# wty-yy/go2_rl_gym

Hardware: AMD Instinct MI355X
Metric: env-steps/sec at 4096 envs (go2 flat); 1/2/4/8-GPU scaling (higher is better)
Workload: dtype f32; 1 GPU; task=go2 flat terrain (go2_flat), num_envs=4096 per GPU, full PPO iteration = 24 rollout steps + GAE + 5 epochs x 4 mini-batches; num_envs_per_gpu=4096, num_steps_per_env=24, parallelism=env-sharded dp1

## Files before the change

### go2_rl_gym_amd/csrc/go2nn_bx3.h

```cpp
#pragma once

#ifndef GO2_EMU
typedef __bf16 bf16x8 __attribute__((ext_vector_type(8)));
typedef __bf16 bf16x2 __attribute__((ext_vector_type(2)));
typedef unsigned u32x2 __attribute__((ext_vector_type(2)));
typedef unsigned u32x4 __attribute__((ext_vector_type(4)));
#endif

#define BX3_BK 16
#ifndef BX3_DA
#define BX3_DA(TM) ((TM) == 1 ? 4 : 2)
#endif
#define BX3_SGB_VALU 5
#define BX3_TILE_BYTES 12288

#ifdef GO2_EMU
#define BX3_HD
#else
#define BX3_HD __host__ __device__
#endif
BX3_HD static inline long long bx3_image_bytes(int rows, int con) { return (long long)((rows + 127) / 128) * ((con + BX3_BK - 1) / BX3_BK) * BX3_TILE_BYTES; }

struct Bx3Prob {
  const float* A; const unsigned char* B; float* C; const float* bias; const float* Y; float* part;
  int M, N, K, lda, ldc, nbm, nbn, c_vec, nkt;
  const float* Bf; int ldb;
  float* wpart; int kx;
};
struct Bx3Args { Bx3Prob p[2]; int ntiles0, ntiles; long long* stamps; int wg_M, wg_rows; };
struct Bx3SplitJob { const float* w; unsigned char* img; int N, K; };
struct Bx3SplitArgs { Bx3SplitJob j[GO2NN_MAX_SPLIT_JOBS]; int njobs; };

#ifndef GO2_EMU
__device__ __forceinline__ unsigned bx3_pk(float a, float b) { f32x2 v = {a, b}; return __builtin_bit_cast(unsigned, __builtin_convertvector(v, bf16x2)); }
__device__ __forceinline__ float bx3_lo(unsigned p) { return __builtin_bit_cast(float, p << 16); }
__device__ __forceinline__ float bx3_hi(unsigned p) { return __builtin_bit_cast(float, p & 0xffff0000u); }
__device__ __forceinline__ void bx3_split4(const f32x4& x, u32x2& h, u32x2& m, u32x2& l) {
  h[0] = bx3_pk(x[0], x[1]); h[1] = bx3_pk(x[2], x[3]);
  const float r0 = x[0] - bx3_lo(h[0]), r1 = x[1] - bx3_hi(h[0]), r2 = x[2] - bx3_lo(h[1]), r3 = x[3] - bx3_hi(h[1]);
  m[0] = bx3_pk(r0, r1); m[1] = bx3_pk(r2, r3);
  const float s0 = r0 - bx3_lo(m[0]), s1 = r1 - bx3_hi(m[0]), s2 = r2 - bx3_lo(m[1]), s3 = r3 - bx3_hi(m[1]);
  l[0] = bx3_pk(s0, s1); l[1] = bx3_pk(s2, s3);
}

__global__ void __launch_bounds__(256) go2nn_bx3_split_kernel(const Bx3SplitArgs sa) {
  const int job = blockIdx.y >> 1, tr = blockIdx.y & 1;
  const Bx3SplitJob& j = sa.j[job];
  const int rows = tr ? j.K : j.N, con = tr ? j.N : j.K;
  const int nrt = (rows + 127) / 128, nkt = (con + BX3_BK - 1) / BX3_BK;
  const long long id = (long long)blockIdx.x * 256 + threadIdx.x;
  if (id >= (long long)nrt * nkt * 256) return;
  const int chunk = (int)(id & 1), r = (int)(id >> 1) & 127, tile = (int)(id >> 8), kt = tile % nkt, rt = tile / nkt;
  const int row = rt * 128 + r, c0 = kt * BX3_BK + chunk * 8;
  f32x4 v[2];
#pragma unroll
  for (int e = 0; e < 8; ++e) {
    const int c = c0 + e;
    const bool in = row < rows && c < con;
    const int rr = min(row, rows - 1), cc = min(c, con - 1);
    const float x = tr ? j.w[(size_t)cc * j.K + rr] : j.w[(size_t)rr * j.K + cc];
    v[e >> 2][e & 3] = in ? x : 0.f;
  }
  u32x2 h0, m0, l0, h1, m1, l1;
  bx3_split4(v[0], h0, m0, l0); bx3_split4(v[1], h1, m1, l1);
  unsigned char* img = j.img + (tr ? bx3_image_bytes(j.N, j.K) : 0) + (size_t)tile * BX3_TILE_BYTES + r * 32 + ((chunk ^ ((r >> 3) & 1)) << 4);
  *reinterpret_cast<u32x4*>(img) = u32x4{h0[0], h0[1], h1[0], h1[1]};
  *reinterpret_cast<u32x4*>(img + 4096) = u32x4{m0[0], m0[1], m1[0], m1[1]};
  *reinterpret_cast<u32x4*>(img + 8192) = u32x4{l0[0], l0[1], l1[0], l1[1]};
}

__device__ __forceinline__ int lane_pos_x(int i, int gk) { return i * 2 + gk; }
template <int OFF> __device__ __forceinline__ void bx3_dsr128(u32x4& d, unsigned addr) { asm volatile("ds_read_b128 %0, %1 offset:%2" : "=v"(d) : "v"(addr), "i"(OFF) : "memory"); }
template <int TM> struct Bx3Frags {
  u32x4 a[TM][2], b[2][2];
  __device__ __forceinline__ void opaque() {
#pragma unroll
    for (int p = 0; p < 2; ++p) {
#pragma unroll
      for (int t = 0; t < TM; ++t) g3_opaque(a[t][p]);
#pragma unroll
      for (int t = 0; t < 2; ++t) g3_opaque(b[t][p]);
    }
  }
};
template <int TM, int EPI, bool WG = false>
__global__ void __launch_bounds__(256, 2) go2nn_bx3_kernel(const Bx3Args ga) {
  static_assert(!WG || (TM == 2 && EPI == EPI_STORE), "weight-gradient mode: 128 x 128 tiles, plain store");
  static_assert(EPI != EPI_DELU_WG || (TM == 2 && !WG), "input gradient + the weight gradient below: 128-row tiles");
  constexpr int BM = 64 * TM, BN = 128, BK = BX3_BK, TN = 2;
  constexpr int AP = BM * 32, BP = 4096, BOFF = 3 * AP, STAGE = 3 * AP + 3 * BP, LOOP_LDS = 2 * STAGE, EPI_LDS = 4 * 32 * 32 * TN * 4;
  using SA = G3Stage<BM, true, BK>;
  using FR = Bx3Frags<TM>;
  __shared__ __attribute__((aligned(16))) unsigned char lds[LOOP_LDS > EPI_LDS ? LOOP_LDS : EPI_LDS];
  const int tid = threadIdx.x, lane = tid & 63, wave = tid >> 6, i = lane & 31, gk = lane >> 5, wm = wave & 1, wn = wave >> 1;
  int t = blockIdx.x, pi, slice = 0;
  const int n0 = ga.ntiles0, n1 = ga.ntiles - ga.ntiles0;
  if constexpr (WG) {
    const int xcd = t & 7, idx = t >> 3;
    slice = (idx / ga.ntiles) * 8 + xcd; t = idx % ga.ntiles;
    pi = t >= n0 ? 1 : 0; t -= pi ? n0 : 0;
  } else if (((n0 | n1) & 7) == 0) { const int x = t & 7, j = t >> 3, c0 = n0 >> 3, c1 = n1 >> 3; pi = j >= c0 ? 1 : 0; t = pi ? x * c1 + (j - c0) : x * c0 + j; }
  else { pi = t >= n0 ? 1 : 0; t -= pi ? n0 : 0; }
  const Bx3Prob& g = ga.p[pi];
  const int bm = t / g.nbn, bn = t - bm * g.nbn;
  const int row0 = bm * BM, col0 = bn * BN;
  const int nk = WG ? (ga.wg_rows + BK - 1) / BK : g.nkt;
  const int m0 = slice * ga.wg_rows;
  float* const Cout = g.C + (WG ? (size_t)slice * g.M * g.N : 0);

#ifdef GM3_STAMPS
  long long st_[6] = {0, 0, 0, 0, 0, 0};
  const long long wall0_ = wall_clock64();
#endif
  G3_T(0);
  f32x16 acc[TM][TN];
#pragma unroll
  for (int a = 0; a < TM; ++a)
#pragma unroll
    for (int b = 0; b < TN; ++b)
#pragma unroll
      for (int r = 0; r < 16; ++r) acc[a][b][r] = 0.f;

  constexpr int CT = 32 * TN, LPR = CT / 4, RPI = 64 / LPR, NI = 32 / RPI;
  const int lc = (lane % LPR) * 4, lr = lane / LPR;
  const int col = col0 + wn * CT + lc;
  const bool cv = g.c_vec != 0 && col + 3 < g.N;
  float4 bias4 = make_float4(0.f, 0.f, 0.f, 0.f);
  if (EPI == EPI_BIAS_ELU || EPI == EPI_BIAS) {
    const int c1 = min(col, g.N - 1), c2 = min(col + 1, g.N - 1), c3 = min(col + 2, g.N - 1), c4 = min(col + 3, g.N - 1);
    bias4 = make_float4(g.bias[c1], g.bias[c2], g.bias[c3], g.bias[c4]);
  }
  float4 y4[EPI == EPI_DELU_COLSUM ? TM : 1][EPI == EPI_DELU_COLSUM ? NI : 1];
  auto load_y = [&](auto a_c) __attribute__((always_inline)) {
    constexpr int A_ = decltype(a_c)::value;
    if constexpr (EPI == EPI_DELU_COLSUM) {
#pragma unroll
      for (int n = 0; n < NI; ++n) {
        const float* q = g.Y + (size_t)min(row0 + wm * 32 * TM + A_ * 32 + lr + n * RPI, g.M - 1) * g.ldc;
        if (cv) y4[A_][n] = *reinterpret_cast<const float4*>(q + col);
        else y4[A_][n] = make_float4(q[min(col, g.N - 1)], q[min(col + 1, g.N - 1)], q[min(col + 2, g.N - 1)], q[min(col + 3, g.N - 1)]);
      }
    }
  };

  const int kx = EPI == EPI_DELU_WG ? g.kx : 0;
  const bool two = kx > 32;
  const int xj = tid & 31, xjt = (tid >> 5) & 1, xhk = (tid >> 6) & 1, xkb = tid >> 7;
  float xv[EPI == EPI_DELU_WG ? 4 : 1][8];
  auto issue_xv = [&]() __attribute__((always_inline)) {
    if constexpr (EPI == EPI_DELU_WG) {
      if (xjt == 0 || two) {
        const float* const xq = g.Bf + min(xjt * 32 + xj, kx - 1);
#pragma unroll
        for (int rt = 0; rt < 4; ++rt)
#pragma unroll
          for (int e = 0; e < 8; ++e) xv[rt][e] = xq[(size_t)gm_opaque(min(row0 + rt * 32 + 16 * xkb + (e & 3) + 8 * (e >> 2) + 4 * xhk, g.M - 1)) * g.ldb];
      }
    }
  };
  SA sa; sa.init(g.A, g.lda, row0, g.M, WG ? 4 : g.K, tid);
  constexpr int DA = BX3_DA(TM);
  f32x4 ba[DA][WG ? 4 : SA::P]; u32x4 bb[3];
  const int scol = tid & 127, skg = tid >> 7;
  unsigned voa[WG ? 8 : 1], vob[WG ? 8 : 1];
  if constexpr (WG) {
#pragma unroll
    for (int j = 0; j < 8; ++j) {
      voa[j] = (unsigned)(((skg * 8 + j) * g.lda + row0 + scol) * 4);
      vob[j] = col0 + scol < g.N ? (unsigned)(((skg * 8 + j) * g.ldb + col0 + scol) * 4) : 0x7ffffff0u;
    }
  }
  auto wg_rsrc = [&](const float* base, int ld, int mrow) __attribute__((always_inline)) {
    const long long left = (long long)(ga.wg_M - mrow) * ld * 4;
    const float* p0 = base + (size_t)mrow * ld;
    const unsigned lo = __builtin_amdgcn_readfirstlane((unsigned)(uintptr_t)p0), hi = __builtin_amdgcn_readfirstlane((unsigned)((uintptr_t)p0 >> 32));
    const unsigned nb = __builtin_amdgcn_readfirstlane(left > 0 ? (unsigned)(left < 0x7fffffe0ll ? left : 0x7fffffe0ll) : 0u);
    return __builtin_amdgcn_make_buffer_rsrc(reinterpret_cast<void*>(((uintptr_t)hi << 32) | lo), 0, nb, 0x00020000);
  };
  auto issue_wg = [&](int kt, f32x4 (&w)[WG ? 4 : SA::P]) __attribute__((always_inline)) {
    if constexpr (WG) {
      const int mrow = m0 + kt * BK;
      const auto ra = wg_rsrc(g.A, g.lda, mrow), rb = wg_rsrc(g.Bf, g.ldb, mrow);
#pragma unroll
      for (int j = 0; j < 8; ++j) {
        w[j >> 2][j & 3] = __builtin_bit_cast(float, __builtin_amdgcn_raw_buffer_load_b32(ra, voa[j], 0, 0));
        w[2 + (j >> 2)][j & 3] = __builtin_bit_cast(float, __builtin_amdgcn_raw_buffer_load_b32(rb, vob[j], 0, 0));
      }
    }
  };
  auto commit_wg = [&](int stage, int kt, const f32x4 (&w)[WG ? 4 : SA::P]) __attribute__((always_inline)) {
    if constexpr (WG) {
      unsigned char* st = lds + stage * STAGE + scol * 32 + ((skg ^ ((scol >> 3) & 1)) << 4);
      const f32x4 a0 = w[0], a1 = w[1];
      u32x2 h0, m0_, l0, h1, m1, l1;
      bx3_split4(a0, h0, m0_, l0); bx3_split4(a1, h1, m1, l1);
      *reinterpret_cast<u32x4*>(st) = u32x4{h0[0], h0[1], h1[0], h1[1]};
      *reinterpret_cast<u32x4*>(st + AP) = u32x4{m0_[0], m0_[1], m1[0], m1[1]};
      *reinterpret_cast<u32x4*>(st + 2 * AP) = u32x4{l0[0], l0[1], l1[0], l1[1]};
      bx3_split4(w[2], h0, m0_, l0); bx3_split4(w[3], h1, m1, l1);
      *reinterpret_cast<u32x4*>(st + BOFF) = u32x4{h0[0], h0[1], h1[0], h1[1]};
      *reinterpret_cast<u32x4*>(st + BOFF + BP) = u32x4{m0_[0], m0_[1], m1[0], m1[1]};
      *reinterpret_cast<u32x4*>(st + BOFF + 2 * BP) = u32x4{l0[0], l0[1], l1[0], l1[1]};
    }
  };
  const unsigned char* bimg = WG ? nullptr : g.B + (size_t)bn * nk * BX3_TILE_BYTES + tid * 16;
  auto issue_b = [&](int kt) __attribute__((always_inline)) {
    if constexpr (WG) return;
    const unsigned char* s = bimg + (size_t)kt * BX3_TILE_BYTES;
#pragma unroll
    for (int p = 0; p < 3; ++p) bb[p] = *reinterpret_cast<const u32x4*>(s + p * 4096);
  };
  const int kq = tid & 3, srow = tid >> 2;
  const unsigned st_off = (unsigned)(srow * 32 + (((kq >> 1) ^ ((srow >> 3) & 1)) << 4) + ((kq & 1) << 3));
  auto commit = [&](auto fix_c, int stage, int kt, const f32x4 (&ba)[SA::P]) __attribute__((always_inline)) {
    constexpr bool FIX = decltype(fix_c)::value;
    unsigned char* st = lds + stage * STAGE;
#pragma unroll
    for (int p = 0; p < SA::P; ++p) {
      f32x4 v = ba[p];
      if (FIX) {
        const int k = kt * BK + sa.lead, sh = k - min(k, g.K - 4);
#pragma unroll
        for (int e = 0; e < 4; ++e) { float tv = 0.f;
#pragma unroll
          for (int q = 0; q < 4; ++q) tv = (q == e + sh) ? ba[p][q] : tv;
          v[e] = k + e < g.K ? tv : 0.f; }
      }
      u32x2 h, m, l; bx3_split4(v, h, m, l);
      unsigned char* d = st + st_off + p * (64 * 32);
      *reinterpret_cast<u32x2*>(d) = h; *reinterpret_cast<u32x2*>(d + AP) = m; *reinterpret_cast<u32x2*>(d + 2 * AP) = l;
    }
#pragma unroll
    for (int p = 0; p < 3; ++p) *reinterpret_cast<u32x4*>(st + BOFF + p * 4096 + tid * 16) = bb[p];
  };
  const unsigned lbase = (unsigned)(uintptr_t)lds;
  const unsigned fch = (unsigned)((gk ^ ((i >> 3) & 1)) << 4);
  const unsigned fa = lbase + (unsigned)((wm * 32 * TM + i) * 32) + fch, fb = lbase + (unsigned)(BOFF + (wn * 64 + i) * 32) + fch;
  FR f0, f1; u32x4 la[TM], lb[2];
  auto read_frags = [&](auto stage_c, FR& f) __attribute__((always_inline)) {
    constexpr int SOFF = decltype(stage_c)::value * STAGE;
    g3_for<0, TM>([&](auto a_c) __attribute__((always_inline)) { constexpr int A = decltype(a_c)::value; bx3_dsr128<SOFF + 2 * AP + A * 32 * 32>(la[A], fa); });
    g3_for<0, 2>([&](auto b_c) __attribute__((always_inline)) { constexpr int B = decltype(b_c)::value; bx3_dsr128<SOFF + 2 * BP + B * 32 * 32>(lb[B], fb); });
    g3_for<0, 2>([&](auto p_c) __attribute__((always_inline)) {
      constexpr int P = decltype(p_c)::value;
      g3_for<0, TM>([&](auto a_c) __attribute__((always_inline)) { constexpr int A = decltype(a_c)::value; bx3_dsr128<SOFF + P * AP + A * 32 * 32>(f.a[A][P], fa); });
      g3_for<0, 2>([&](auto b_c) __attribute__((always_inline)) { constexpr int B = decltype(b_c)::value; bx3_dsr128<SOFF + P * BP + B * 32 * 32>(f.b[B][P], fb); });
    });
  };
  auto mfmas = [&](auto q0_c, auto q1_c, const FR& f) __attribute__((always_inline)) {
    constexpr int PA[6] = {2, 0, 1, 1, 0, 0}, PB[6] = {0, 2, 1, 0, 1, 0};
    g3_for<decltype(q0_c)::value, decltype(q1_c)::value>([&](auto q_c) __attribute__((always_inline)) {
      constexpr int Q = decltype(q_c)::value;
#pragma unroll
      for (int a = 0; a < TM; ++a)
#pragma unroll
        for (int b = 0; b < TN; ++b) {
          const u32x4 av = PA[Q] == 2 ? la[a] : f.a[a][PA[Q] & 1], bv = PB[Q] == 2 ? lb[b] : f.b[b][PB[Q] & 1];
          acc[a][b] = __builtin_amdgcn_mfma_f32_32x32x16_bf16(__builtin_bit_cast(bf16x8, av), __builtin_bit_cast(bf16x8, bv), acc[a][b], 0, 0, 0);
        }
    });
  };
  auto lo_opaque = [&]() __attribute__((always_inline)) {
#pragma unroll
    for (int t = 0; t < TM; ++t) g3_opaque(la[t]);
#pragma unroll
    for (int t = 0; t < 2; ++t) g3_opaque(lb[t]);
  };

  const bool ragged = !WG && (g.K & (BK - 1)) != 0;
  const int nkp = ragged ? nk - 1 : nk;
  auto tile = [&](auto cur_c, auto set_c, const bool MORE, int kt) __attribute__((always_inline)) {
    constexpr int CUR = decltype(cur_c)::value, SET = decltype(set_c)::value;
    auto& a_ld = ba[SET]; auto& a_st = ba[(SET + 1) % DA];
    FR& fc = CUR ? f1 : f0; FR& fn = CUR ? f0 : f1;
    { const int k2 = min(kt + DA, nkp - 1); if constexpr (WG) issue_wg(k2, a_ld); else sa.issue(k2 * BK, a_ld); }
    g3_wait_lgkm<0>();
    fc.opaque(); lo_opaque();
    mfmas(G3Int<0>{}, G3Int<3>{}, fc);
    if (MORE) {
      if constexpr (WG) commit_wg(CUR ^ 1, kt + 1, a_st); else commit(G3Int<0>{}, CUR ^ 1, kt + 1, a_st);
      issue_b(min(kt + 2, nkp - 1));
#pragma unroll
      for (int q = 0; q < 6 * TM; ++q) {
        __builtin_amdgcn_sched_group_barrier(0x008, 1, 0);
        __builtin_amdgcn_sched_group_barrier(0x002, BX3_SGB_VALU, 0);
        __builtin_amdgcn_sched_group_barrier(0x200, 1, 0);
        if (q < 3) __builtin_amdgcn_sched_group_barrier(0x020, 1, 0);
      }
      __builtin_amdgcn_sched_barrier(0);
      __syncthreads();
      read_frags(G3Int<CUR ^ 1>{}, fn);
      __builtin_amdgcn_sched_barrier(0);
    }
    mfmas(G3Int<3>{}, G3Int<6>{}, fc);
    __builtin_amdgcn_sched_barrier(0);
  };
  constexpr G3Int<0> I0{}; constexpr G3Int<1> I1{};
  if (nkp > 0) {
    issue_b(0);
    g3_for<0, DA>([&](auto d_c) __attribute__((always_inline)) { constexpr int D_ = decltype(d_c)::value;
      if constexpr (WG) issue_wg(min(D_, nkp - 1), ba[D_]); else sa.issue(min(D_, nkp - 1) * BK, ba[D_]); });
    if constexpr (TM == 2) load_y(G3Int<0>{});
    issue_xv();
    if constexpr (WG) commit_wg(0, 0, ba[0]); else commit(I0, 0, 0, ba[0]);
    if (nkp > 1) issue_b(1);
    __syncthreads();
    read_frags(I0, f0);
    G3_T(1);
    constexpr int G = (DA % 2) ? 2 * DA : DA;
    for (int kt = 0; kt < nkp; kt += G)
      g3_for<0, G>([&](auto j_c) __attribute__((always_inline)) { constexpr int J = decltype(j_c)::value; if (kt + J < nkp) tile(G3Int<J & 1>{}, G3Int<J % DA>{}, kt + J + 1 < nkp, kt + J); });
  } else if constexpr (TM == 2) {
    issue_xv();
    load_y(G3Int<0>{});
  }
  if constexpr (!WG) if (ragged) {
    __syncthreads();
    sa.issue((nk - 1) * BK, ba[0]); issue_b(nk - 1);
    commit(I1, 0, nk - 1, ba[0]);
    __syncthreads();
    read_frags(I0, f0);
    g3_wait_lgkm<0>();
    f0.opaque(); lo_opaque();
    mfmas(G3Int<0>{}, G3Int<6>{}, f0);
  }
  G3_T(2);
  __syncthreads();
  G3_T(3);

  if constexpr (EPI == EPI_DELU_WG) {
#if defined(GM3_STAMPS) && defined(WG_T3)
#define WG_STAMP(n) do { if (WG_T3 == (n)) G3_T(3); if (WG_T5 == (n)) G3_T(5); } while (0)
#else
#define WG_STAMP(n) do { } while (0)
#endif
    const int rw = row0 + wm * 64, cw = col0 + wn * 64;
    const bool xon = xjt == 0 || two;
    float y[2][2][16];
#pragma unroll
    for (int a = 0; a < 2; ++a)
#pragma unroll
      for (int r = 0; r < 16; ++r) {
        const float* q = g.Y + (size_t)gm_opaque(min(rw + a * 32 + (r & 3) + 8 * (r >> 2) + 4 * gk, g.M - 1)) * g.ldc;
#pragma unroll
        for (int b = 0; b < 2; ++b) y[a][b][r] = q[min(cw + b * 32 + i, g.N - 1)];
      }
    WG_STAMP(1);
    float cs[2] = {0.f, 0.f};
#pragma unroll
    for (int a = 0; a < 2; ++a)
#pragma unroll
      for (int r = 0; r < 16; ++r) {
        const bool in = rw + a * 32 + (r & 3) + 8 * (r >> 2) + 4 * gk < g.M;
#pragma unroll
        for (int b = 0; b < 2; ++b) {
          const float v = gm_keep(acc[a][b][r] * (y[a][b][r] > 0.f ? 1.f : y[a][b][r] + 1.f), in);
          acc[a][b][r] = v; cs[b] += v;
        }
      }
#pragma unroll
    for (int b = 0; b < 2; ++b) {
      const float t2 = cs[b] + __shfl_xor(cs[b], 32);
      const int c = cw + b * 32 + i;
      if (gk == 0 && c < g.N && (bm * 2 + wm) * 64 < g.M) g.part[(size_t)(bm * 2 + wm) * g.N + c] = t2;
    }
    if (g.C) {
      float* wl = reinterpret_cast<float*>(lds) + wave * (32 * CT);
#pragma unroll
      for (int a = 0; a < 2; ++a) {
#pragma unroll
        for (int b = 0; b < 2; ++b)
#pragma unroll
          for (int r = 0; r < 16; ++r) {
            const int row = (r & 3) + 8 * (r >> 2) + 4 * gk, cc = b * 32 + i;
            wl[row * CT + (cc ^ (gk << 5 & (CT - 1)))] = acc[a][b][r];
          }
#pragma unroll
        for (int n = 0; n < NI; ++n) {
          const int lrow = lr + n * RPI, row = rw + a * 32 + lrow;
          const float4 v = *reinterpret_cast<const float4*>(wl + lrow * CT + (lc ^ ((lrow >> 2 & 1) << 5 & (CT - 1))));
          if (row < g.M) {
            float* o = g.C + (size_t)row * g.ldc + col;
            if (cv) *reinterpret_cast<float4*>(o) = v;
            else { if (col < g.N) o[0] = v.x; if (col + 1 < g.N) o[1] = v.y; if (col + 2 < g.N) o[2] = v.z; if (col + 3 < g.N) o[3] = v.w; }
          }
        }
      }
      __syncthreads();
    }
    if (xon) {
      const bool in = xjt * 32 + xj < kx;
#pragma unroll
      for (int rt = 0; rt < 4; ++rt) {
// ... 143 lines not shown
```

### go2_rl_gym_amd/csrc/go2nn_impl.cpp

```cpp
#include <math.h>
#include <stdint.h>
#include <stdio.h>
#include <string.h>
#include <stdlib.h>
#include <algorithm>
#include <vector>

#include "../../include/go2nn.h"

#ifndef GO2_EMU
#include <hip/hip_runtime.h>
#endif

static thread_local char g_err[256] = "";
#define FAIL(code, ...) do { snprintf(g_err, sizeof(g_err), __VA_ARGS__); return (code); } while (0)

#define NN_ROWS 32
#define NN_LD (GO2NN_MAX_WIDTH + 4)
#ifndef NN_THREADS
#define NN_THREADS 512
#endif
#define NN_WAVES (NN_THREADS / 64)
#define NN3_LDS 163840
#define nn3_pitch(width) (((width) + 31) / 32 * 64 + 16)
// ... 564 lines not shown
#endif
  return 0;
}

int go2nn_linear_backward_weight(const float* gz, const float* x, float* dw, float* workspace, int32_t M, int32_t C, int32_t Kin, void* stream) {
  if (!gz || !x || !dw || !workspace || !lin_check(M, C, Kin)) FAIL(GO2NN_EINVAL, "linear backward (weight): bad argument");
#ifdef GO2_EMU
  (void)stream; (void)workspace;
  for (int64_t i = 0; i < (int64_t)C * Kin; ++i) dw[i] = 0.f;
  for (int m = 0; m < M; ++m) for (int c = 0; c < C; ++c) { const float gv = gz[(int64_t)m * C + c]; for (int k = 0; k < Kin; ++k) dw[(int64_t)c * Kin + k] = fmaf(gv, x[(int64_t)m * Kin + k], dw[(int64_t)c * Kin + k]); }
#else
  GemmArgs g; memset(&g, 0, sizeof(g));
  int tm, tn, s, kc; wgrad_shape(M, C, Kin, &tm, &tn, &s, &kc);
  g.A = gz; g.B = x; g.C = s > 1 ? workspace : dw; g.M = C; g.N = Kin; g.K = M; g.lda = C; g.ldb = Kin; g.ldc = Kin;
  const bool vec = (C % 4 == 0) && (Kin % 4 == 0) && aligned16(gz) && aligned16(x);
  g.kchunk = kc; g.c_split_stride = (long long)C * Kin; g.nbm = cdiv(C, 64 * tm); g.nbn = cdiv(Kin, 64 * tn);
  g.c_vec = (Kin % 4 == 0) && aligned16(g.C);
  gemm_dispatch<false, false, EPI_STORE>(tm, tn, g, s, vec, (hipStream_t)stream);
  HIPCHK(hipGetLastError());
  if (s > 1) { const Go2nnSumJob job = {workspace, dw, s, C * Kin}; return go2nn_sum_rows(&job, 1, stream); }
#endif
  return 0;
}

#ifdef GO2NN_STAMPS
int go2nn_policy_act_stamped(const Go2nnMlp* actor, const float* actor_packed, const Go2nnMlp* critic, const float* critic_packed,
                             const float* obs, const float* critic_obs, const float* std_, const float* eps, float* a_out, void* stamps, int32_t N, void* stream) {
  NNArgs a; memset(&a, 0, sizeof(a));
  if (!describe(actor, &a.net[0], nullptr) || !describe(critic, &a.net[1], nullptr)) return GO2NN_EINVAL;
  a.net[0].packed = actor_packed; net_io(a.net[0], obs, N, nullptr); a.net[1].packed = critic_packed; net_io(a.net[1], critic_obs, N, nullptr);
  a.std_ = std_; a.eps = eps; a.a_out = a_out; a.y = (float*)stamps; a.N = N; a.A = a.net[0].out_dim; a.mode = 1;
  return run(a, 2, stream);
}
#endif

}

#ifndef GO2_EMU
#ifdef GM3_STAMPS
static long long* g_gemm3_stamps = nullptr;
extern "C" void go2nn_debug_gemm3_stamps(long long* p) { g_gemm3_stamps = p; }
#define GM3_SET_STAMPS(a) (a).stamps = g_gemm3_stamps
#else
#define GM3_SET_STAMPS(a) do { } while (0)
#endif
template <bool BKC, int EPI>
static int gemm3_launch(int tm, int tn, int bk, const Gemm3Args& a, hipStream_t st) {
  const dim3 grid(a.ntiles), blk(256);
  if (tm == 1 && tn == 2 && bk == 32)      hipLaunchKernelGGL((go2nn_gemm3_kernel<1, 2, BKC, EPI, 32>), grid, blk, 0, st, a);
  else if (tm == 1 && tn == 1 && bk == 32) hipLaunchKernelGGL((go2nn_gemm3_kernel<1, 1, BKC, EPI, 32>), grid, blk, 0, st, a);
  else FAIL(GO2NN_EINVAL, "gemm3: no kernel for tile %d x %d x %d", tm, tn, bk);
  HIPCHK(hipGetLastError());
  return 0;
}
template <int EPI>
static int bx3_launch(int tm, const Bx3Args& a, hipStream_t st) {
  const dim3 grid(a.ntiles), blk(256);
  if (tm == 3) { if constexpr (EPI == EPI_BIAS_ELU || EPI == EPI_BIAS) hipLaunchKernelGGL((go2nn_bx3_kernel<3, EPI>), grid, blk, 0, st, a); else FAIL(GO2NN_EINVAL, "bx3: no 192-row tile for this epilogue"); }
  else if (tm == 2) hipLaunchKernelGGL((go2nn_bx3_kernel<2, EPI>), grid, blk, 0, st, a);
  else              hipLaunchKernelGGL((go2nn_bx3_kernel<1, EPI>), grid, blk, 0, st, a);
  HIPCHK(hipGetLastError());
  return 0;
}
static inline int bx3_tm(int M, int N0, int N1, int tm_max) {
  static const char* const env = getenv("GO2NN_BX3_TM");
  if (env && env[0] >= '1' && env[0] <= '0' + tm_max) return env[0] - '0';
  int best = 1; double best_eff = -1.0;
  for (int tm = 1; tm <= tm_max; ++tm) {
    const long long tiles = (long long)cdiv(M, 64 * tm) * (cdiv(N0, 128) + (N1 ? cdiv(N1, 128) : 0)), slots = tm == 1 ? 768 : 512;
    const double eff = (double)tiles / (double)((tiles + slots - 1) / slots * slots);
    if (eff >= best_eff - 1e-9) { best_eff = eff > best_eff ? eff : best_eff; best = tm; }
  }
  return best;
}
template <bool VECA, bool VECB>
static int wgrad3_launch2(int ta, int tn, const WgArgs& a, hipStream_t st) {
  const dim3 grid(a.tiles * a.nsplit), blk(256);
  if (tn == 4) hipLaunchKernelGGL((go2nn_wgrad_kernel<2, 4, VECA, VECB, 6>), grid, blk, 0, st, a);
  else              hipLaunchKernelGGL((go2nn_wgrad_kernel<2, 2, VECA, VECB, 8>), grid, blk, 0, st, a);
  HIPCHK(hipGetLastError());
  return 0;
}
#endif
static int wgrad3_group_shape(const Go2nnBwdWJob* jobs, int njobs, int* ta, int* tn, int* tiles_of, int* nsplit, int* rows) {
  if (!jobs || njobs < 1 || njobs > GO2NN_MAX_GROUP) return 0;
  *tn = 4; *ta = 2;
  bool split = true; int t128 = 0;
  int kin_sum = 0, kin_pad = 0;
  for (int j = 0; j < njobs; ++j) {
    if (!lin_check(jobs[j].M, jobs[j].C, jobs[j].Kin) || jobs[j].M != jobs[0].M || jobs[j].C < 2 || jobs[j].Kin < 4) return 0;
    if (jobs[j].Kin % 128) *tn = 2;
    if (!jobs[j].split || jobs[j].C % 128) split = false;
    t128 += (jobs[j].C / 128) * cdiv(jobs[j].Kin, 128); kin_sum += jobs[j].Kin; kin_pad += cdiv(jobs[j].Kin, 128) * 128;
  }
#ifndef GO2_EMU
  if (kin_pad > 2 * kin_sum) split = false;
  static const bool no_wg_split = getenv("GO2NN_WG_SPLIT") && atoi(getenv("GO2NN_WG_SPLIT")) == 0;
  if (split && t128 >= 8 && !no_wg_split) {
    *ta = 9;
    for (int j = 0; j < njobs; ++j) tiles_of[j] = (jobs[j].C / 128) * cdiv(jobs[j].Kin, 128);
    wgrad3_shape(jobs[0].M, t128, nsplit, rows);
    *rows = (*rows + BX3_BK - 1) / BX3_BK * BX3_BK;
    return t128;
  }
#endif
  int tiles = 0;
  for (int j = 0; j < njobs; ++j) { tiles_of[j] = cdiv(jobs[j].C, 32 * *ta) * cdiv(jobs[j].Kin, 32 * *tn); tiles += tiles_of[j]; }
  wgrad3_shape(jobs[0].M, tiles, nsplit, rows);
  return tiles;
}

extern "C" {

int64_t go2nn_split_weights_bytes(int32_t N, int32_t K) {
  if (N <= 0 || K <= 0 || N > 4096 || K > 4096) FAIL(GO2NN_EINVAL, "split image: bad shape");
  return bx3_image_bytes(N, K) + bx3_image_bytes(K, N);
}

int go2nn_split_weights(const Go2nnSplitJob* jobs, int32_t njobs, void* stream) {
  if (!jobs || njobs < 1 || njobs > GO2NN_MAX_SPLIT_JOBS) FAIL(GO2NN_EINVAL, "split weights: 1..%d jobs", GO2NN_MAX_SPLIT_JOBS);
  for (int j = 0; j < njobs; ++j) if (!jobs[j].w || !jobs[j].image || jobs[j].N <= 0 || jobs[j].K <= 0 || jobs[j].N > 4096 || jobs[j].K > 4096 || ((uintptr_t)jobs[j].image & 15)) FAIL(GO2NN_EINVAL, "split weights: bad job %d", j);
#ifdef GO2_EMU
  return 0;
#else
  Bx3SplitArgs a; memset(&a, 0, sizeof(a)); a.njobs = njobs;
  long long most = 0;
  for (int j = 0; j < njobs; ++j) { a.j[j].w = jobs[j].w; a.j[j].img = (unsigned char*)jobs[j].image; a.j[j].N = jobs[j].N; a.j[j].K = jobs[j].K;
    most = std::max(most, std::max(bx3_image_bytes(jobs[j].N, jobs[j].K), bx3_image_bytes(jobs[j].K, jobs[j].N)) / 48); }
  hipLaunchKernelGGL(go2nn_bx3_split_kernel, dim3((unsigned)cdiv((int)most, 256), 2 * njobs), dim3(256), 0, (hipStream_t)stream, a);
  HIPCHK(hipGetLastError());
  return 0;
#endif
}

int go2nn_linear_elu_forward_group(const Go2nnFwdJob* jobs, int32_t njobs, void* stream) {
  if (!jobs || njobs < 1 || njobs > GO2NN_MAX_GROUP) FAIL(GO2NN_EINVAL, "forward group: 1..%d jobs", GO2NN_MAX_GROUP);
  for (int j = 0; j < njobs; ++j) if (!jobs[j].x || !jobs[j].w || !jobs[j].b || !jobs[j].y || !lin_check(jobs[j].M, jobs[j].N, jobs[j].K)) FAIL(GO2NN_EINVAL, "forward group: bad job %d", j);
  const int act = jobs[0].act;
  if (act != 0 && act != 1) FAIL(GO2NN_EINVAL, "forward group: act 0 (ELU) or 1 (none)");
  for (int j = 1; j < njobs; ++j) if (jobs[j].act != act) FAIL(GO2NN_EINVAL, "forward group: every job of a group carries the same activation flag");
#ifdef GO2_EMU
  for (int j = 0; j < njobs; ++j) {
    if (!act) { const int rc = go2nn_linear_elu_forward(jobs[j].x, jobs[j].w, jobs[j].b, jobs[j].y, jobs[j].M, jobs[j].K, jobs[j].N, stream); if (rc) return rc; continue; }
    const Go2nnFwdJob& q = jobs[j];
    for (int m = 0; m < q.M; ++m) for (int n = 0; n < q.N; ++n) {
      float acc = 0.f;
      for (int k = 0; k < q.K; ++k) acc = fmaf(q.x[(int64_t)m * q.K + k], q.w[(int64_t)n * q.K + k], acc);
      q.y[(int64_t)m * q.N + n] = acc + q.b[n];
    }
  }
  return 0;
#else
  if (jobs[0].w_split && jobs[njobs - 1].w_split && jobs[0].K >= 4 && jobs[njobs - 1].K >= 4) {
    Bx3Args a; memset(&a, 0, sizeof(a));
    const int tm = bx3_tm(jobs[0].M, jobs[0].N, njobs == 2 ? jobs[1].N : 0, 3);
    for (int j = 0; j < njobs; ++j) {
      Bx3Prob& g = a.p[j]; const Go2nnFwdJob& q = jobs[j];
      g.A = q.x; g.B = (const unsigned char*)q.w_split; g.C = q.y; g.bias = q.b; g.M = q.M; g.N = q.N; g.K = q.K; g.lda = q.K; g.ldc = q.N;
      g.nbm = cdiv(q.M, 64 * tm); g.nbn = cdiv(q.N, 128); g.nkt = cdiv(q.K, BX3_BK); g.c_vec = (q.N % 4 == 0) && aligned16(q.y);
      (j ? a.ntiles : a.ntiles0) = g.nbm * g.nbn;
    }
    a.ntiles = njobs == 2 ? a.ntiles0 + a.ntiles : a.ntiles0;
    GM3_SET_STAMPS(a);
    return act ? bx3_launch<EPI_BIAS>(tm, a, (hipStream_t)stream) : bx3_launch<EPI_BIAS_ELU>(tm, a, (hipStream_t)stream);
  }
  int tm, tn, bk; gemm3_tile(jobs[0].N, &tm, &tn, &bk);
  if (njobs == 2) { int tm1, tn1, bk1; gemm3_tile(jobs[1].N, &tm1, &tn1, &bk1);
    if (tm1 != tm || tn1 != tn || bk1 != bk) { const int rc = go2nn_linear_elu_forward_group(jobs, 1, stream); return rc ? rc : go2nn_linear_elu_forward_group(jobs + 1, 1, stream); } }
  for (int j = 0; j < njobs; ++j) if (jobs[j].K < 4) {
    if (act) FAIL(GO2NN_EINVAL, "forward group: a layer without activation needs K >= 4");
    for (int i = 0; i < njobs; ++i) { const int rc = go2nn_linear_elu_forward(jobs[i].x, jobs[i].w, jobs[i].b, jobs[i].y, jobs[i].M, jobs[i].K, jobs[i].N, stream); if (rc) return rc; }
    return 0; }
  Gemm3Args a; memset(&a, 0, sizeof(a));
  for (int j = 0; j < njobs; ++j) {
    Gemm3Prob& g = a.p[j]; const Go2nnFwdJob& q = jobs[j];
    g.A = q.x; g.B = q.w; g.C = q.y; g.bias = q.b; g.M = q.M; g.N = q.N; g.K = q.K; g.lda = q.K; g.ldb = q.K; g.ldc = q.N;
    g.nbm = cdiv(q.M, 64 * tm); g.nbn = cdiv(q.N, 64 * tn); g.c_vec = (q.N % 4 == 0) && aligned16(q.y);
    (j ? a.ntiles : a.ntiles0) = g.nbm * g.nbn;
  }
  a.ntiles = njobs == 2 ? a.ntiles0 + a.ntiles : a.ntiles0;
  GM3_SET_STAMPS(a);
  return act ? gemm3_launch<true, EPI_BIAS>(tm, tn, bk, a, (hipStream_t)stream) : gemm3_launch<true, EPI_BIAS_ELU>(tm, tn, bk, a, (hipStream_t)stream);
// ... 50 lines not shown
      float acc = 0.f;
      for (int c = 0; c < q.C; ++c) acc = fmaf(q.gz[(int64_t)m * q.C + c], q.w[(int64_t)c * q.Kin + k], acc);
      if (!plain) { const float y = q.y_prev[m * ld + k]; acc *= y > 0.f ? 1.f : y + 1.f; q.workspace[k] += acc; }
      q.gz_prev[m * ld + k] = acc;
    }
  }
  return 0;
#else
  if (jobs[0].w_split && jobs[njobs - 1].w_split && jobs[0].C >= 4 && jobs[njobs - 1].C >= 4) {
    Bx3Args a; memset(&a, 0, sizeof(a));
    const int tm = fused ? 2 : bx3_tm(jobs[0].M, jobs[0].Kin, njobs == 2 ? jobs[1].Kin : 0, 2);
    for (int j = 0; j < njobs; ++j) {
      Bx3Prob& g = a.p[j]; const Go2nnBwdInJob& q = jobs[j];
      g.Bf = q.x_in; g.ldb = q.ldx ? q.ldx : q.Kx; g.kx = q.Kx; g.wpart = q.dw_workspace;
      g.A = q.gz; g.B = (const unsigned char*)q.w_split + bx3_image_bytes(q.C, q.Kin); g.C = q.gz_prev; g.Y = q.y_prev; g.part = q.workspace;
      g.M = q.M; g.N = q.Kin; g.K = q.C; g.lda = q.C; g.ldc = q.ld ? q.ld : q.Kin;
      g.nbm = cdiv(q.M, 64 * tm); g.nbn = cdiv(q.Kin, 128); g.nkt = cdiv(q.C, BX3_BK); g.c_vec = (q.Kin % 4 == 0) && (g.ldc % 4 == 0) && aligned16(q.gz_prev) && (plain || aligned16(q.y_prev));
      (j ? a.ntiles : a.ntiles0) = g.nbm * g.nbn;
    }
    a.ntiles = njobs == 2 ? a.ntiles0 + a.ntiles : a.ntiles0;
    GM3_SET_STAMPS(a);
    if (fused) {
      hipLaunchKernelGGL((go2nn_bx3_kernel<2, EPI_DELU_WG>), dim3(a.ntiles), dim3(256), 0, (hipStream_t)stream, a);
      HIPCHK(hipGetLastError());
      return 0;
    }
    return plain ? bx3_launch<EPI_STORE>(tm, a, (hipStream_t)stream) : bx3_launch<EPI_DELU_COLSUM>(tm, a, (hipStream_t)stream);
  }
  int tm, tn, bk; gemm3_tile(jobs[0].Kin, &tm, &tn, &bk);
  if (njobs == 2) { int tm1, tn1, bk1; gemm3_tile(jobs[1].Kin, &tm1, &tn1, &bk1);
    if (tm1 != tm || tn1 != tn || bk1 != bk) { const int rc = go2nn_linear_backward_input_group(jobs, 1, stream); return rc ? rc : go2nn_linear_backward_input_group(jobs + 1, 1, stream); } }
  for (int j = 0; j < njobs; ++j) if (jobs[j].C < 4 || jobs[j].Kin < 4 || jobs[j].Kin % 4) {
    for (int i = 0; i < njobs; ++i) if (jobs[i].ld) FAIL(GO2NN_EINVAL, "pitched input gradient on the fp32-MFMA kernels: C >= 4 and Kin a multiple of 4");
    if (plain) FAIL(GO2NN_EINVAL, "plain input gradient on the fp32-MFMA kernels: C >= 4 and Kin a multiple of 4 (the split-operand kernel takes any Kin)");
    for (int i = 0; i < njobs; ++i) {
      const Go2nnBwdInJob& q = jobs[i];
      GemmArgs g; memset(&g, 0, sizeof(g));
      int tm1, tn1; gemm_tile(q.M, q.Kin, &tm1, &tn1); tm1 = 1;
      g.A = q.gz; g.B = q.w; g.C = q.gz_prev; g.Y = q.y_prev; g.part = q.workspace; g.M = q.M; g.N = q.Kin; g.K = q.C; g.lda = q.C; g.ldb = q.Kin; g.ldc = q.Kin;
      const bool vec = (q.C % 4 == 0) && (q.Kin % 4 == 0) && aligned16(q.gz) && aligned16(q.w);
      g.kchunk = cdiv(q.C, GM_BK) * GM_BK; g.nbm = cdiv(q.M, gm_tile_rows(tm1)); g.nbn = cdiv(q.Kin, 64 * tn1);
      g.c_vec = (q.Kin % 4 == 0) && aligned16(q.gz_prev) && aligned16(q.y_prev);
      gemm_dispatch<true, false, EPI_DELU_COLSUM>(tm1, tn1, g, 1, vec, (hipStream_t)stream);
      HIPCHK(hipGetLastError());
    }
    return 0; }
  Gemm3Args a; memset(&a, 0, sizeof(a));
  for (int j = 0; j < njobs; ++j) {
    Gemm3Prob& g = a.p[j]; const Go2nnBwdInJob& q = jobs[j];
    g.A = q.gz; g.B = q.w; g.C = q.gz_prev; g.Y = q.y_prev; g.part = q.workspace; g.M = q.M; g.N = q.Kin; g.K = q.C; g.lda = q.C; g.ldb = q.Kin; g.ldc = q.ld ? q.ld : q.Kin;
    g.nbm = cdiv(q.M, 64 * tm); g.nbn = cdiv(q.Kin, 64 * tn); g.c_vec = (q.Kin % 4 == 0) && (g.ldc % 4 == 0) && aligned16(q.gz_prev) && (plain || aligned16(q.y_prev));
    (j ? a.ntiles : a.ntiles0) = g.nbm * g.nbn;
  }
  a.ntiles = njobs == 2 ? a.ntiles0 + a.ntiles : a.ntiles0;
  GM3_SET_STAMPS(a);
  return plain ? gemm3_launch<false, EPI_STORE>(tm, tn, bk, a, (hipStream_t)stream) : gemm3_launch<false, EPI_DELU_COLSUM>(tm, tn, bk, a, (hipStream_t)stream);
#endif
}

int32_t go2nn_linear_backward_weight_group_rows(const Go2nnBwdWJob* jobs, int32_t njobs) {
#ifdef GO2_EMU
  if (!jobs || njobs < 1 || njobs > GO2NN_MAX_GROUP) FAIL(GO2NN_EINVAL, "weight-gradient group: 1..%d jobs", GO2NN_MAX_GROUP);
  return 1;
#else
  int ta, tn, tiles_of[GO2NN_MAX_GROUP], nsplit, rows;
  if (!wgrad3_group_shape(jobs, njobs, &ta, &tn, tiles_of, &nsplit, &rows)) FAIL(GO2NN_EINVAL, "weight-gradient group: 1..%d jobs with one M, C >= 2, Kin >= 4", GO2NN_MAX_GROUP);
  return nsplit;
#endif
}

int go2nn_linear_backward_weight_group(const Go2nnBwdWJob* jobs, int32_t njobs, void* stream) {
  int ta, tn, tiles_of[GO2NN_MAX_GROUP], nsplit, rows;
  const int tiles = wgrad3_group_shape(jobs, njobs, &ta, &tn, tiles_of, &nsplit, &rows);
  if (!tiles) FAIL(GO2NN_EINVAL, "weight-gradient group: 1..%d jobs with one M, C >= 2, Kin >= 4", GO2NN_MAX_GROUP);
  for (int j = 0; j < njobs; ++j) if (!jobs[j].gz || !jobs[j].x || !jobs[j].workspace || (jobs[j].ldx != 0 && jobs[j].ldx < jobs[j].Kin)) FAIL(GO2NN_EINVAL, "weight-gradient group: bad job %d", j);
#ifdef GO2_EMU
  for (int j = 0; j < njobs; ++j) {
    const Go2nnBwdWJob& q = jobs[j];
    std::vector<float> xd;
    if (q.ldx && q.ldx != q.Kin) { xd.resize((size_t)q.M * q.Kin); for (int m = 0; m < q.M; ++m) memcpy(&xd[(size_t)m * q.Kin], q.x + (size_t)m * q.ldx, q.Kin * sizeof(float)); }
    const int rc = go2nn_linear_backward_weight(q.gz, xd.empty() ? q.x : xd.data(), q.workspace, q.workspace, q.M, q.C, q.Kin, stream); if (rc) return rc; }
  return 0;
#else
  for (int j = 0; j < njobs; ++j) if (jobs[j].ldx && jobs[j].ldx != jobs[j].Kin && ta != 9) FAIL(GO2NN_EINVAL, "weight-gradient group: a pitched x (ldx) on the split-operand kernel only (C in whole 128-row tiles, >= 8 tiles)");
  WgArgs a; memset(&a, 0, sizeof(a));
  if (ta == 9) {
    Bx3Args b; memset(&b, 0, sizeof(b));
    for (int j = 0; j < njobs; ++j) {
      Bx3Prob& g = b.p[j]; const Go2nnBwdWJob& q = jobs[j];
      g.A = q.gz; g.lda = q.C; g.Bf = q.x; g.ldb = q.ldx ? q.ldx : q.Kin; g.C = q.workspace; g.ldc = q.Kin; g.M = q.C; g.N = q.Kin; g.K = rows;
      g.nbm = q.C / 128; g.nbn = cdiv(q.Kin, 128); g.c_vec = aligned16(q.workspace) && (q.Kin % 4 == 0);
    }
    b.ntiles0 = tiles_of[0]; b.ntiles = tiles; b.wg_M = jobs[0].M; b.wg_rows = rows;
    hipLaunchKernelGGL((go2nn_bx3_kernel<2, EPI_STORE, true>), dim3(tiles * nsplit), dim3(256), 0, (hipStream_t)stream, b);
    HIPCHK(hipGetLastError());
    return 0;
  }
  bool veca = true, vecb = true;
  for (int j = 0; j < njobs; ++j) {
    WgProb& g = a.p[j]; const Go2nnBwdWJob& q = jobs[j];
    g.G = q.gz; g.X = q.x; g.part = q.workspace; g.C = q.C; g.Kin = q.Kin; g.ntc = cdiv(q.C, 32 * ta); g.ntk = cdiv(q.Kin, 32 * tn);
    veca = veca && (q.C % ta == 0) && (((uintptr_t)q.gz & (4 * ta - 1)) == 0);
    vecb = vecb && (q.Kin % tn == 0) && (((uintptr_t)q.x & (4 * tn - 1)) == 0);
  }
  a.M = jobs[0].M; a.rows_per_slice = rows; a.nsplit = nsplit; a.tiles0 = tiles_of[0]; a.tiles = tiles;
  hipStream_t st = (hipStream_t)stream;
  return veca ? (vecb ? wgrad3_launch2<true, true>(ta, tn, a, st) : wgrad3_launch2<true, false>(ta, tn, a, st))
              : (vecb ? wgrad3_launch2<false, true>(ta, tn, a, st) : wgrad3_launch2<false, false>(ta, tn, a, st));
#endif
}

}

extern "C" {

static int ppo_heads_ok(int B, int A, int K) { return B > 0 && A >= 1 && A <= HB_MAX_C && K >= 4 && K <= 256 && (K & 3) == 0; }
int32_t go2nn_ppo_heads_cols(int32_t A, int32_t K) {
  if (!ppo_heads_ok(1, A, K)) FAIL(GO2NN_EINVAL, "ppo heads: 1 <= A <= %d, K a multiple of 4 up to 256", HB_MAX_C);
  return ppo_heads_cols(A, K);
}
int32_t go2nn_ppo_heads_rows(int32_t B, int32_t A, int32_t K) {
  if (!ppo_heads_ok(B, A, K)) FAIL(GO2NN_EINVAL, "ppo heads: bad shape");
#ifdef GO2_EMU
  return 1;
#else
  int q, rows, nwg; ppo_heads_shape(B, K, &q, &rows, &nwg); return nwg;
#endif
}
int go2nn_ppo_heads(const Go2nnPpoHeads* h, void* stream) {
  if (!h || !ppo_heads_ok(h->B, h->A, h->K)) FAIL(GO2NN_EINVAL, "ppo heads: bad shape");
  const void* ptrs[] = {h->y_a, h->y_c, h->w_mu, h->b_mu, h->w_v, h->b_v, h->std, h->actions, h->old_mu, h->old_sigma, h->old_logp, h->adv, h->old_values, h->returns, h->gz_a, h->gz_c, h->partials};
  for (const void* q : ptrs) if (!q) FAIL(GO2NN_EINVAL, "ppo heads: null pointer");
  const int B = h->B, A = h->A, K = h->K;
#ifdef GO2_EMU
  (void)stream;
  const float LOG2PI = 1.8378770664093453f, invB = 1.f / (float)B, lo = 1.f - h->clip, hi = 1.f + h->clip;
  const int split = (h->surrogate_split > 0 && h->surrogate_split < B) ? h->surrogate_split : 0;
  const float w_head = split ? 1.f / (float)split : invB, w_tail = split ? 1.f / (float)(B - split) : invB;
  float* S = h->partials; const int nc = ppo_heads_cols(A, K);
  for (int i = 0; i < nc; ++i) S[i] = 0.f;
  float* pa = S + PH_NSTAT + A; float* pc = pa + (size_t)(A + 1) * K + A;
  for (int c = 0; c < A; ++c) { S[3] += 0.5f + 0.5f * LOG2PI + logf(h->std[c]); S[PH_NSTAT + c] = -h->entropy_coef / h->std[c]; }
  for (int r = 0; r < B; ++r) {
    const float* ya = h->y_a + (size_t)r * K; const float* yc = h->y_c + (size_t)r * K;
    float mu[HB_MAX_C], v = h->b_v[0], lp = 0.f, kl = 0.f;
    for (int k = 0; k < K; ++k) v = fmaf(yc[k], h->w_v[k], v);
    for (int c = 0; c < A; ++c) {
      float m = h->b_mu[c]; for (int k = 0; k < K; ++k) m = fmaf(ya[k], h->w_mu[(size_t)c * K + k], m);
      mu[c] = m;
      const float sg = h->std[c], d = h->actions[(size_t)r * A + c] - m, so = h->old_sigma[(size_t)r * A + c], dm = h->old_mu[(size_t)r * A + c] - m, isg2 = 1.f / (sg * sg);
      lp += -d * d * (0.5f * isg2) - logf(sg) - 0.5f * LOG2PI; kl += logf(sg / so + 1e-5f) + (so * so + dm * dm) * (0.5f * isg2) - 0.5f;
    }
    const float ad = h->adv[r], ratio = expf(lp - h->old_logp[r]), rc = fminf(fmaxf(ratio, lo), hi), in = (ratio >= lo && ratio <= hi) ? 1.f : 0.f;
    const float s1 = -ad * ratio, s2 = -ad * rc, sur = fmaxf(s1, s2), w = s1 > s2 ? 1.f : (s1 < s2 ? in : 0.5f + 0.5f * in), wr = (!split || r < split) ? w_head : w_tail, g_lp = -ad * w * ratio * wr;
    const float tv = h->old_values[r], rt = h->returns[r], dv = v - tv;
    float vl, gv;
    if (h->use_clipped_value_loss) {
      const float dc = fminf(fmaxf(dv, -h->clip), h->clip), vin = (dv >= -h->clip && dv <= h->clip) ? 1.f : 0.f, vc = tv + dc;
      const float l1 = (v - rt) * (v - rt), l2 = (vc - rt) * (vc - rt); vl = fmaxf(l1, l2);
      const float g1 = 2.f * (v - rt), g2 = 2.f * (vc - rt) * vin; gv = l1 > l2 ? g1 : (l1 < l2 ? g2 : 0.5f * g1 + 0.5f * g2);
    } else { vl = (rt - v) * (rt - v); gv = 2.f * (v - rt); }
    const float gval = h->value_loss_coef * gv * invB;
    S[0] += sur * wr; S[1] += vl * invB; S[2] += kl * invB;
    float gm[HB_MAX_C];
    for (int c = 0; c < A; ++c) { const float sg = h->std[c], d = h->actions[(size_t)r * A + c] - mu[c], isg2 = 1.f / (sg * sg);
      gm[c] = g_lp * d * isg2; S[PH_NSTAT + c] += g_lp * (d * d * isg2 / sg - 1.f / sg); pa[(size_t)(A + 1) * K + c] += gm[c]; }
    for (int k = 0; k < K; ++k) {
      float gx = 0.f; for (int c = 0; c < A; ++c) { gx = fmaf(gm[c], h->w_mu[(size_t)c * K + k], gx); pa[(size_t)c * K + k] = fmaf(gm[c], ya[k], pa[(size_t)c * K + k]); }
      const float oa = gx * (ya[k] > 0.f ? 1.f : ya[k] + 1.f), oc = gval * h->w_v[k] * (yc[k] > 0.f ? 1.f : yc[k] + 1.f);
      h->gz_a[(size_t)r * K + k] = oa; h->gz_c[(size_t)r * K + k] = oc; pa[(size_t)A * K + k] += oa; pc[K + k] += oc; pc[k] = fmaf(gval, yc[k], pc[k]);
    }
    pc[2 * K] += gval;
  }
#else
  PpoHeadsArgs a;
  a.y_a = h->y_a; a.y_c = h->y_c; a.w_mu = h->w_mu; a.b_mu = h->b_mu; a.w_v = h->w_v; a.b_v = h->b_v; a.std_ = h->std; a.actions = h->actions; a.old_mu = h->old_mu;
  a.old_sigma = h->old_sigma; a.old_logp = h->old_logp; a.adv = h->adv; a.old_values = h->old_values; a.returns = h->returns; a.gz_a = h->gz_a; a.gz_c = h->gz_c; a.part = h->partials;
// ... 167 lines not shown
```

Before: 6.808 million env-steps/s.

## Stage weight-gradient operands k-major and read fragments with transposing LDS loads

Adds a transposed-staging variant of the split-bf16 weight-gradient GEMM kernel. Global loads become 128-bit vector buffer loads of contiguous rows, and the data is stored k-major in LDS with an XOR swizzle. Fragments are then read back with ds_read_b64_tr_b16, replacing the scalar per-element 32-bit gathers. The prefetch depth for this path rises to 3 and the main loop gets an unguarded full-group body. The variant is the default whenever every Kin is a multiple of 4, and it adds register pressure and a new swizzle layout that must be correct.

```diff
diff --git a/go2_rl_gym_amd/csrc/go2nn_bx3.h b/go2_rl_gym_amd/csrc/go2nn_bx3.h
--- a/go2_rl_gym_amd/csrc/go2nn_bx3.h
+++ b/go2_rl_gym_amd/csrc/go2nn_bx3.h
@@ -10,6 +10,9 @@
 #define BX3_BK 16
 #ifndef BX3_DA
 #define BX3_DA(TM) ((TM) == 1 ? 4 : 2)
+#endif
+#ifndef BX3_DA_WG
+#define BX3_DA_WG 3
 #endif
 #define BX3_SGB_VALU 5
 #define BX3_TILE_BYTES 12288
@@ -71,6 +74,10 @@
 
 __device__ __forceinline__ int lane_pos_x(int i, int gk) { return i * 2 + gk; }
 template <int OFF> __device__ __forceinline__ void bx3_dsr128(u32x4& d, unsigned addr) { asm volatile("ds_read_b128 %0, %1 offset:%2" : "=v"(d) : "v"(addr), "i"(OFF) : "memory"); }
+template <int OFF> __device__ __forceinline__ void bx3_dsr64tr(u32x2& d, unsigned addr) { asm volatile("ds_read_b64_tr_b16 %0, %1 offset:%2" : "=v"(d) : "v"(addr), "i"(OFF) : "memory"); }
+template <int OFF> __device__ __forceinline__ void bx3_frag_tr(u32x4& d, unsigned a0, unsigned a1) {
+  u32x2 lo, hi; bx3_dsr64tr<OFF>(lo, a0); bx3_dsr64tr<OFF>(hi, a1); d = u32x4{lo[0], lo[1], hi[0], hi[1]};
+}
 template <int TM> struct Bx3Frags {
   u32x4 a[TM][2], b[2][2];
   __device__ __forceinline__ void opaque() {
@@ -83,9 +90,10 @@
     }
   }
 };
-template <int TM, int EPI, bool WG = false>
+template <int TM, int EPI, bool WG = false, bool TR = false>
 __global__ void __launch_bounds__(256, 2) go2nn_bx3_kernel(const Bx3Args ga) {
   static_assert(!WG || (TM == 2 && EPI == EPI_STORE), "weight-gradient mode: 128 x 128 tiles, plain store");
+  static_assert(!TR || WG, "transposed staging: weight-gradient mode only");
   static_assert(EPI != EPI_DELU_WG || (TM == 2 && !WG), "input gradient + the weight gradient below: 128-row tiles");
   constexpr int BM = 64 * TM, BN = 128, BK = BX3_BK, TN = 2;
   constexpr int AP = BM * 32, BP = 4096, BOFF = 3 * AP, STAGE = 3 * AP + 3 * BP, LOOP_LDS = 2 * STAGE, EPI_LDS = 4 * 32 * 32 * TN * 4;
@@ -159,11 +167,22 @@
     }
   };
   SA sa; sa.init(g.A, g.lda, row0, g.M, WG ? 4 : g.K, tid);
-  constexpr int DA = BX3_DA(TM);
+  constexpr int DA = TR ? BX3_DA_WG : BX3_DA(TM);
   f32x4 ba[DA][WG ? 4 : SA::P]; u32x4 bb[3];
   const int scol = tid & 127, skg = tid >> 7;
-  unsigned voa[WG ? 8 : 1], vob[WG ? 8 : 1];
-  if constexpr (WG) {
+  unsigned voa[WG && !TR ? 8 : 1], vob[WG && !TR ? 8 : 1];
+  const int tq = tid & 31, tr0 = tid >> 5;
+  unsigned toa[TR ? 2 : 1], tob[TR ? 2 : 1], tst[TR ? 2 : 1];
+  auto tr_swz = [](int r) __attribute__((always_inline)) { return ((r & 3) << 2) | ((r >> 2) & 3); };
+  if constexpr (TR) {
+#pragma unroll
+    for (int j = 0; j < 2; ++j) {
+      const int r = tr0 + 8 * j;
+      toa[j] = (unsigned)((r * g.lda + row0 + 4 * tq) * 4);
+      tob[j] = col0 + 4 * tq < g.N ? (unsigned)((r * g.ldb + col0 + 4 * tq) * 4) : 0x7ffffff0u;
+      tst[j] = (unsigned)(r * 256 + (((tq >> 1) ^ tr_swz(r)) << 4) + ((tq & 1) << 3));
+    }
+  } else if constexpr (WG) {
 #pragma unroll
     for (int j = 0; j < 8; ++j) {
       voa[j] = (unsigned)(((skg * 8 + j) * g.lda + row0 + scol) * 4);
@@ -178,7 +197,15 @@
     return __builtin_amdgcn_make_buffer_rsrc(reinterpret_cast<void*>(((uintptr_t)hi << 32) | lo), 0, nb, 0x00020000);
   };
   auto issue_wg = [&](int kt, f32x4 (&w)[WG ? 4 : SA::P]) __attribute__((always_inline)) {
-    if constexpr (WG) {
+    if constexpr (TR) {
+      const int mrow = m0 + kt * BK;
+      const auto ra = wg_rsrc(g.A, g.lda, mrow), rb = wg_rsrc(g.Bf, g.ldb, mrow);
+#pragma unroll
+      for (int j = 0; j < 2; ++j) {
+        w[j] = __builtin_bit_cast(f32x4, __builtin_amdgcn_raw_buffer_load_b128(ra, toa[j], 0, 0));
+        w[2 + j] = __builtin_bit_cast(f32x4, __builtin_amdgcn_raw_buffer_load_b128(rb, tob[j], 0, 0));
+      }
+    } else if constexpr (WG) {
       const int mrow = m0 + kt * BK;
       const auto ra = wg_rsrc(g.A, g.lda, mrow), rb = wg_rsrc(g.Bf, g.ldb, mrow);
 #pragma unroll
@@ -189,7 +216,16 @@
     }
   };
   auto commit_wg = [&](int stage, int kt, const f32x4 (&w)[WG ? 4 : SA::P]) __attribute__((always_inline)) {
-    if constexpr (WG) {
+    if constexpr (TR) {
+      unsigned char* st = lds + stage * STAGE;
+#pragma unroll
+      for (int j = 0; j < 4; ++j) {
+        u32x2 h, m, l; bx3_split4(w[j], h, m, l);
+        unsigned char* d = st + tst[j & 1] + (j >> 1) * BOFF;
+        constexpr int PS = AP;
+        *reinterpret_cast<u32x2*>(d) = h; *reinterpret_cast<u32x2*>(d + PS) = m; *reinterpret_cast<u32x2*>(d + 2 * PS) = l;
+      }
+    } else if constexpr (WG) {
       unsigned char* st = lds + stage * STAGE + scol * 32 + ((skg ^ ((scol >> 3) & 1)) << 4);
       const f32x4 a0 = w[0], a1 = w[1];
       u32x2 h0, m0_, l0, h1, m1, l1;
@@ -236,9 +272,32 @@
   const unsigned lbase = (unsigned)(uintptr_t)lds;
   const unsigned fch = (unsigned)((gk ^ ((i >> 3) & 1)) << 4);
   const unsigned fa = lbase + (unsigned)((wm * 32 * TM + i) * 32) + fch, fb = lbase + (unsigned)(BOFF + (wn * 64 + i) * 32) + fch;
+  unsigned tfa[TR ? TM : 1][2], tfb[TR ? 2 : 1][2];
+  if constexpr (TR) {
+    static_assert(AP == BP, "k-major images: 128 columns per operand");
+#pragma unroll
+    for (int h = 0; h < 2; ++h) {
+      const int r = 8 * gk + 4 * h + ((lane >> 2) & 3), cl = (i & 16) + 4 * (lane & 3);
+      auto at = [&](int c) __attribute__((always_inline)) { return lbase + (unsigned)(r * 256 + ((((c + cl) >> 3) ^ tr_swz(r)) << 4) + ((lane & 1) << 3)); };
+#pragma unroll
+      for (int a = 0; a < TM; ++a) tfa[a][h] = at(wm * 32 * TM + a * 32);
+#pragma unroll
+      for (int b = 0; b < 2; ++b) tfb[b][h] = at(wn * 64 + b * 32) + BOFF;
+    }
+  }
   FR f0, f1; u32x4 la[TM], lb[2];
   auto read_frags = [&](auto stage_c, FR& f) __attribute__((always_inline)) {
     constexpr int SOFF = decltype(stage_c)::value * STAGE;
+    if constexpr (TR) {
+      g3_for<0, TM>([&](auto a_c) __attribute__((always_inline)) { constexpr int A = decltype(a_c)::value; bx3_frag_tr<SOFF + 2 * AP>(la[A], tfa[A][0], tfa[A][1]); });
+      g3_for<0, 2>([&](auto b_c) __attribute__((always_inline)) { constexpr int B = decltype(b_c)::value; bx3_frag_tr<SOFF + 2 * BP>(lb[B], tfb[B][0], tfb[B][1]); });
+      g3_for<0, 2>([&](auto p_c) __attribute__((always_inline)) {
+        constexpr int P = decltype(p_c)::value;
+        g3_for<0, TM>([&](auto a_c) __attribute__((always_inline)) { constexpr int A = decltype(a_c)::value; bx3_frag_tr<SOFF + P * AP>(f.a[A][P], tfa[A][0], tfa[A][1]); });
+        g3_for<0, 2>([&](auto b_c) __attribute__((always_inline)) { constexpr int B = decltype(b_c)::value; bx3_frag_tr<SOFF + P * BP>(f.b[B][P], tfb[B][0], tfb[B][1]); });
+      });
+      return;
+    }
     g3_for<0, TM>([&](auto a_c) __attribute__((always_inline)) { constexpr int A = decltype(a_c)::value; bx3_dsr128<SOFF + 2 * AP + A * 32 * 32>(la[A], fa); });
     g3_for<0, 2>([&](auto b_c) __attribute__((always_inline)) { constexpr int B = decltype(b_c)::value; bx3_dsr128<SOFF + 2 * BP + B * 32 * 32>(lb[B], fb); });
     g3_for<0, 2>([&](auto p_c) __attribute__((always_inline)) {
@@ -308,7 +367,11 @@
     read_frags(I0, f0);
     G3_T(1);
     constexpr int G = (DA % 2) ? 2 * DA : DA;
-    for (int kt = 0; kt < nkp; kt += G)
+    int kt = 0;
+    if constexpr (TR)
+      for (; kt + G <= nkp; kt += G)
+        g3_for<0, G>([&](auto j_c) __attribute__((always_inline)) { constexpr int J = decltype(j_c)::value; tile(G3Int<J & 1>{}, G3Int<J % DA>{}, kt + J + 1 < nkp, kt + J); });
+    for (; kt < nkp; kt += G)
       g3_for<0, G>([&](auto j_c) __attribute__((always_inline)) { constexpr int J = decltype(j_c)::value; if (kt + J < nkp) tile(G3Int<J & 1>{}, G3Int<J % DA>{}, kt + J + 1 < nkp, kt + J); });
   } else if constexpr (TM == 2) {
     issue_xv();
diff --git a/go2_rl_gym_amd/csrc/go2nn_impl.cpp b/go2_rl_gym_amd/csrc/go2nn_impl.cpp
--- a/go2_rl_gym_amd/csrc/go2nn_impl.cpp
+++ b/go2_rl_gym_amd/csrc/go2nn_impl.cpp
@@ -670,6 +670,9 @@
   return 0;
 }
 #endif
+#ifndef BX3_WG_MIN_TILES
+#define BX3_WG_MIN_TILES 8
+#endif
 static int wgrad3_group_shape(const Go2nnBwdWJob* jobs, int njobs, int* ta, int* tn, int* tiles_of, int* nsplit, int* rows) {
   if (!jobs || njobs < 1 || njobs > GO2NN_MAX_GROUP) return 0;
   *tn = 4; *ta = 2;
@@ -684,8 +687,12 @@
 #ifndef GO2_EMU
   if (kin_pad > 2 * kin_sum) split = false;
   static const bool no_wg_split = getenv("GO2NN_WG_SPLIT") && atoi(getenv("GO2NN_WG_SPLIT")) == 0;
-  if (split && t128 >= 8 && !no_wg_split) {
-    *ta = 9;
+  static const bool no_wg_tr = getenv("GO2NN_WG_TR") && atoi(getenv("GO2NN_WG_TR")) == 0;
+  static const int min_tiles = getenv("GO2NN_WG_MIN_TILES") ? atoi(getenv("GO2NN_WG_MIN_TILES")) : BX3_WG_MIN_TILES;
+  bool tr = !no_wg_tr;
+  for (int j = 0; j < njobs; ++j) if (jobs[j].Kin % 4) tr = false;
+  if (split && t128 >= min_tiles && !no_wg_split) {
+    *ta = tr ? 10 : 9;
     for (int j = 0; j < njobs; ++j) tiles_of[j] = (jobs[j].C / 128) * cdiv(jobs[j].Kin, 128);
     wgrad3_shape(jobs[0].M, t128, nsplit, rows);
     *rows = (*rows + BX3_BK - 1) / BX3_BK * BX3_BK;
@@ -902,9 +909,9 @@
     const int rc = go2nn_linear_backward_weight(q.gz, xd.empty() ? q.x : xd.data(), q.workspace, q.workspace, q.M, q.C, q.Kin, stream); if (rc) return rc; }
   return 0;
 #else
-  for (int j = 0; j < njobs; ++j) if (jobs[j].ldx && jobs[j].ldx != jobs[j].Kin && ta != 9) FAIL(GO2NN_EINVAL, "weight-gradient group: a pitched x (ldx) on the split-operand kernel only (C in whole 128-row tiles, >= 8 tiles)");
+  for (int j = 0; j < njobs; ++j) if (jobs[j].ldx && jobs[j].ldx != jobs[j].Kin && ta < 9) FAIL(GO2NN_EINVAL, "weight-gradient group: a pitched x (ldx) on the split-operand kernel only (C in whole 128-row tiles, >= 8 tiles)");
   WgArgs a; memset(&a, 0, sizeof(a));
-  if (ta == 9) {
+  if (ta >= 9) {
     Bx3Args b; memset(&b, 0, sizeof(b));
     for (int j = 0; j < njobs; ++j) {
       Bx3Prob& g = b.p[j]; const Go2nnBwdWJob& q = jobs[j];
@@ -912,7 +919,9 @@
       g.nbm = q.C / 128; g.nbn = cdiv(q.Kin, 128); g.c_vec = aligned16(q.workspace) && (q.Kin % 4 == 0);
     }
     b.ntiles0 = tiles_of[0]; b.ntiles = tiles; b.wg_M = jobs[0].M; b.wg_rows = rows;
-    hipLaunchKernelGGL((go2nn_bx3_kernel<2, EPI_STORE, true>), dim3(tiles * nsplit), dim3(256), 0, (hipStream_t)stream, b);
+    GM3_SET_STAMPS(b);
+    if (ta == 10) hipLaunchKernelGGL((go2nn_bx3_kernel<2, EPI_STORE, true, true>), dim3(tiles * nsplit), dim3(256), 0, (hipStream_t)stream, b);
+    else          hipLaunchKernelGGL((go2nn_bx3_kernel<2, EPI_STORE, true>), dim3(tiles * nsplit), dim3(256), 0, (hipStream_t)stream, b);
     HIPCHK(hipGetLastError());
     return 0;
   }
```

After: 6.830 million env-steps/s, median of 6. About the same (+0.3%).
